# xiaoyeli/superlu_dist

Measured on AMD Instinct MI355X. Metric: LU factorization GFLOP/s (pdgstrf3d) + solve time, higher is better.
Workload: dtype f64

## Files before the change

__graft_entry__.py:

```python
import os, subprocess, sys

ROOT = os.path.dirname(os.path.abspath(__file__))
sys.path.insert(0, ROOT)
sys.path.insert(0, os.path.join(ROOT, "tests"))


def build():
    subprocess.check_call(["make", "-C", os.path.join(ROOT, "superlu_dist_amd", "csrc")])
    subprocess.check_call(["make", "-C", os.path.join(ROOT, "examples")])
    subprocess.check_call(["make", "-C", os.path.join(ROOT, "oracle")])
    ref_cfg = "/root/reference/SRC/include/superlu_dist_config.h"
    if os.path.isdir("/root/reference/SRC") and not os.path.exists(ref_cfg):
        print("build(): " + ref_cfg + " is absent (cmake-generated): the real reference is NOT built here; oracle/_ref* stay as they are", file=sys.stderr)
    if os.path.exists(ref_cfg):
        subprocess.check_call(["make", "-s", "-C", os.path.join(ROOT, "oracle", "ref")])
        subprocess.check_call(["make", "-s", "-C", os.path.join(ROOT, "oracle", "ref"), "ref64", "-j8"])
        if os.path.exists("/opt/conda/lib/libmkl_rt.so"):
            subprocess.check_call(["make", "-s", "-C", os.path.join(ROOT, "oracle", "ref"), "ref_mkl", "-j8"])
    import superlu_dist_amd
    from superlu_dist_amd import _lib
    _lib.load()


def smoke():
# ... 31 lines not shown
```

include/superlu_dist_amd.h:

```cpp
#ifndef SUPERLU_DIST_AMD_H
#define SUPERLU_DIST_AMD_H

#include <stdint.h>

#ifdef __cplusplus
extern "C" {
#endif

typedef int32_t sluamd_int_t;

#define SLUAMD_OK 0
#define SLUAMD_EINVAL (-1)
#define SLUAMD_ENODEVICE (-2)
#define SLUAMD_EHIP (-3)
#define SLUAMD_ENOMEM (-4)
#define SLUAMD_ESTRUCT (-5)

typedef struct sluamd_dLUview {
    int64_t n;
    int32_t nsupers;
    const sluamd_int_t *xsup;
    int32_t nprow, npcol, npdep;
    int32_t myrow, mycol, myzlayer;
    sluamd_int_t **Lrowind_bc_ptr;
// ... 83 lines not shown
int sluamd_pzgstrf3d(sluamd_handle_t h, double thresh, int *info);
int sluamd_zCopyLU2Host(sluamd_handle_t h, const sluamd_zLUview_t *lu);
int sluamd_pzgstrs3d(sluamd_handle_t h, sluamd_doublecomplex *x, int64_t ldx, int32_t nrhs);

#define SLUAMD_NOTRANS 0
#define SLUAMD_TRANS   1
#define SLUAMD_CONJ    2
int sluamd_pdgstrs3d_trans(sluamd_handle_t h, int trans, double *x, int64_t ldx, int32_t nrhs);
int sluamd_pdgstrs3d_trans_dev(sluamd_handle_t h, int trans, double *d_x, int64_t ldx, int32_t nrhs);
int sluamd_pzgstrs3d_trans(sluamd_handle_t h, int trans, sluamd_doublecomplex *x, int64_t ldx, int32_t nrhs);
int sluamd_pzgstrs3d_trans_dev(sluamd_handle_t h, int trans, sluamd_doublecomplex *d_x, int64_t ldx, int32_t nrhs);

void sluamd_dDestroyLUHandle(sluamd_handle_t h);

int sluamd_get_stats(sluamd_handle_t h, sluamd_stats_t *out);
int sluamd_setup_times(sluamd_handle_t h, char *buf, int32_t cap);
#define SLUAMD_PLAN_COLS 20
int sluamd_plan_table(sluamd_handle_t h, double *buf, int64_t cap_rows, int64_t *rows);
const char *sluamd_last_error(void);
int sluamd_device_count(void);
int64_t sluamd_device_pool_trim(int dev);
int sluamd_device_pci_bus_id(int dev, char *buf, int len);

typedef struct sluamd_symb_s *sluamd_symb_t;

int sluamd_dsymbfact(sluamd_symb_t *s, int64_t n, const sluamd_int_t *rowptr, const sluamd_int_t *colind,
                     const sluamd_int_t *perm_c, int32_t relax, int32_t maxsup, sluamd_int_t *perm_c_out);
int sluamd_dsymbfact_unsym(sluamd_symb_t *s, int64_t n, const sluamd_int_t *rowptr, const sluamd_int_t *colind,
                           const sluamd_int_t *perm_c, int32_t relax, int32_t maxsup, sluamd_int_t *perm_c_out);
int sluamd_order_nd(int64_t n, const sluamd_int_t *rowptr, const sluamd_int_t *colind, int32_t leaf, sluamd_int_t *perm_c);
// ... 106 lines not shown
```

superlu_dist_amd/_lib.py:

```python
import ctypes as C
import os

_HERE = os.path.dirname(os.path.abspath(__file__))
_SO = os.environ.get("SLUAMD_LIB") or os.path.join(_HERE, "libsluamd.so")

int_t = C.c_int32
P_int = C.POINTER(C.c_int32)
P_dbl = C.POINTER(C.c_double)


class LUView(C.Structure):
    _fields_ = [("n", C.c_int64), ("nsupers", C.c_int32), ("xsup", P_int),
                ("nprow", C.c_int32), ("npcol", C.c_int32), ("npdep", C.c_int32),
                ("myrow", C.c_int32), ("mycol", C.c_int32), ("myzlayer", C.c_int32),
                ("Lrowind_bc_ptr", C.POINTER(P_int)), ("Lnzval_bc_ptr", C.POINTER(P_dbl)),
                ("Ufstnz_br_ptr", C.POINTER(P_int)), ("Unzval_br_ptr", C.POINTER(P_dbl))]


class ForestView(C.Structure):
    _fields_ = [("maxLvl", C.c_int32), ("myTreeIdxs", P_int), ("myZeroTrIdxs", P_int),
                ("numForests", C.c_int32), ("nNodes", P_int), ("nodeList", C.POINTER(P_int))]


class Options(C.Structure):
# ... 69 lines not shown
    L.sluamd_dCreateLUHandleFromSymb.argtypes = [C.POINTER(C.c_void_p), C.c_void_p, P_int, P_int, P_dbl, P_int, C.POINTER(Options)]
    L.sluamd_dCreateLUHandleFromSymbGrid.argtypes = [C.POINTER(C.c_void_p), C.c_void_p, P_int, P_int, P_dbl, P_int, C.POINTER(Options),
                                                     P_int, C.c_void_p]
    L.sluamd_zCreateLUHandleFromSymbGrid.argtypes = [C.POINTER(C.c_void_p), C.c_void_p, P_int, P_int, C.c_void_p, P_int, C.POINTER(Options),
                                                     P_int, C.c_void_p]
    L.sluamd_dSetValues.argtypes = [C.c_void_p, C.POINTER(LUView)]
    L.sluamd_pdgstrf3d.argtypes = [C.c_void_p, C.c_double, P_int]
    L.sluamd_factor_info.argtypes = [C.c_void_p, P_int, P_int]
    L.sluamd_dCopyLU2Host.argtypes = [C.c_void_p, C.POINTER(LUView)]
    L.sluamd_pdgstrs3d.argtypes = [C.c_void_p, P_dbl, C.c_int64, C.c_int32]
    L.sluamd_pdgstrs3d_dev.argtypes = [C.c_void_p, C.c_void_p, C.c_int64, C.c_int32]
    L.sluamd_pdgstrs3d_dist.argtypes = [C.c_void_p, C.c_void_p, C.c_int64, C.c_int32, C.c_int64, C.c_int64, P_int, P_int]
    L.sluamd_pzgstrs3d_dist.argtypes = L.sluamd_pdgstrs3d_dist.argtypes
    L.sluamd_dDestroyLUHandle.argtypes = [C.c_void_p]
    L.sluamd_get_stats.argtypes = [C.c_void_p, C.POINTER(Stats)]
    L.sluamd_mfma_selftest.argtypes = [P_dbl, P_dbl, P_dbl]
    L.sluamd_dResetValues.argtypes = [C.c_void_p]
    L.sluamd_zCreateLUHandle.argtypes = L.sluamd_dCreateLUHandle.argtypes
    L.sluamd_zCreateLUHandleGrid.argtypes = L.sluamd_dCreateLUHandleGrid.argtypes
    L.sluamd_zSetValues.argtypes = [C.c_void_p, C.POINTER(LUView)]
    L.sluamd_zCopyLU2Host.argtypes = [C.c_void_p, C.POINTER(LUView)]
    L.sluamd_pzgstrf3d.argtypes = [C.c_void_p, C.c_double, P_int]
    L.sluamd_pzgstrs3d.argtypes = [C.c_void_p, C.c_void_p, C.c_int64, C.c_int32]
    L.sluamd_zCreateLUHandleFromSymb.argtypes = [C.POINTER(C.c_void_p), C.c_void_p, P_int, P_int, C.c_void_p, P_int, C.POINTER(Options)]
    L.sluamd_symb_partition.argtypes = [C.c_void_p, C.c_int32, P_int]
    L.sluamd_symb_grid_footprint.argtypes = [C.c_void_p, C.c_int32, C.c_int32, C.c_int32, P_int, C.POINTER(C.c_int64), C.POINTER(C.c_int64), C.POINTER(C.c_int64)]
    L.sluamd_set_profile.argtypes = [C.c_void_p, C.c_int]
    L.sluamd_setup_times.argtypes = [C.c_void_p, C.c_char_p, C.c_int32]
    L.sluamd_poisson3d.argtypes = [C.c_int32, C.c_int32, C.c_int32, P_int, P_int, P_dbl]
    L.sluamd_poisson3d.restype = C.c_int64
# ... 53 lines not shown
```

superlu_dist_amd/csrc/sluamd_api.cpp:

```cpp
#include <algorithm>
#include <cstdint>
#include <cstdlib>
#include <cstring>
#include "sluamd_comm.h"
#include "sluamd_plan.h"
#include "sluamd_refine.h"

using namespace sluamd;

namespace sluamd {

static int ensure_pinned(Handle *H)
{
    if (H->h_pinned) return 0;
    size_t want = (size_t) 64 << 20;
    if (const char *v = getenv("SLUAMD_PINNED_BYTES")) want = std::max<size_t>(256, (size_t) atoll(v) & ~(size_t) 15);
    HIPCHK(hipHostMalloc(&H->h_pinned, want, hipHostMallocDefault));
    H->pinned_bytes = want;
    return 0;
}

static int copy_values(Handle *H, const sluamd_dLUview_t *lu, int dir)
{
    const HostStruct &hs = H->hs;
// ... 620 lines not shown
                    double b = 0.0;
                    for (size_t a = zl + 1; a < H->forest_nodes.size(); ++a)
                        for (int k : H->forest_nodes[a]) {
                            if (H->grid.kcol(k) == H->grid.c) b += (double) (esz * H->hs.lval_len[k]);
                            if (H->grid.krow(k) == H->grid.r) b += (double) (esz * H->hs.uval_len[k]);
                        }
                    r[15] = send ? b : -b;
                }
            }
        }
    }
    *rows = n;
    return 0;
}

int sluamd_get_stats(sluamd_handle_t h, sluamd_stats_t *out)
{
    if (!h || !out) return SLUAMD_EINVAL;
    *out = h->H.st;
    return 0;
}

int sluamd_dCreateLUHandleFromSymb(sluamd_handle_t *out, sluamd_symb_t s, const sluamd_int_t *rowptr, const sluamd_int_t *colind,
                                   const double *nzval, const sluamd_int_t *perm_c_final, const sluamd_options_t *opt)
{
    return create_from_symb(out, s, rowptr, colind, nzval, perm_c_final, opt, Grid{}, nullptr, nullptr, false);
}

int sluamd_zCreateLUHandleFromSymb(sluamd_handle_t *out, sluamd_symb_t s, const sluamd_int_t *rowptr, const sluamd_int_t *colind,
                                   const sluamd_doublecomplex *nzval, const sluamd_int_t *perm_c_final, const sluamd_options_t *opt)
// ... 58 lines not shown
```

superlu_dist_amd/csrc/sluamd_factor.cpp:

```cpp
#include <algorithm>
#include <cstring>
#include "sluamd_comm.h"
#include "sluamd_plan.h"

namespace sluamd {

static void ev_begin(Handle *H, std::vector<std::pair<hipEvent_t, hipEvent_t>> &v, size_t &used, hipStream_t s)
{
    if (!H->profile) return;
    if (used == v.size()) { hipEvent_t a, b; hipEventCreate(&a); hipEventCreate(&b); v.emplace_back(a, b); }
    hipEventRecord(v[used].first, s);
}
static void ev_end(Handle *H, std::vector<std::pair<hipEvent_t, hipEvent_t>> &v, size_t &used, hipStream_t s)
{
    if (!H->profile) return;
    hipEventRecord(v[used].second, s);
    ++used;
}
static double ev_sum(std::vector<std::pair<hipEvent_t, hipEvent_t>> &v, size_t used)
{
    double tot = 0;
    for (size_t i = 0; i < used; ++i) { float ms = 0; hipEventElapsedTime(&ms, v[i].first, v[i].second); tot += ms; }
    return tot;
}
// ... 377 lines not shown
    return 0;
}

static hipEvent_t red_wait_event(const Handle *H, int64_t lend, int64_t uend)
{
    for (auto &e : H->red_events)
        if ((lend < 0 || e.lend >= lend) && (uend < 0 || e.uend >= uend)) return e.ev;
    return H->red_events.empty() ? nullptr : H->red_events.back().ev;
}

int run_factor(Handle *H, double thresh, int *info)
{
    HIPCHK(hipSetDevice(H->device));
    const Grid &g = H->grid;
    if (g.size() > 1 && !H->comm) { set_error("handle of a multi-rank grid has no communicator"); return SLUAMD_EINVAL; }
    int init[8] = {0x7fffffff, 0, 0, 0, 0, 0, 0, 0};
    HIPCHK(hipMemcpyAsync(H->d_info, init, sizeof(init), hipMemcpyHostToDevice, H->stream));
    H->st.num_launches = 0; H->st.schur_launches = 0; H->st.schur_tiles = 0;
    H->profile = H->opt.verbose >= 2 || H->env.profile;
    H->ev_schur_used = H->ev_panel_used = H->ev_xchg_used = H->ev_red_used = 0;
    H->schur_rec.clear();
    H->ev_pool_used = 0;
    H->red_pool_used = 0; H->red_events.clear();
    HIPCHK(hipEventRecord(H->ev0, H->stream));
    int rc = 0;
    for (size_t zl = 0; zl < H->sched.size(); ++zl) {
        if (H->z_active[zl]) {
            rc = run_factor_sched(H, H->sched[zl], thresh);
            if (rc) return rc;
        }
        if (g.Pz > 1) {
            ev_begin(H, H->ev_red, H->ev_red_used, H->stream);
            rc = reduce_ancestors(H, (int) zl);
            ev_end(H, H->ev_red, H->ev_red_used, H->stream);
            if (rc) return rc;
        }
    }
    if (H->red_all) { HIPCHK(hipStreamWaitEvent(H->stream, H->red_all, 0)); H->red_events.clear(); }
    HIPCHK(hipEventRecord(H->ev1, H->stream));
    int res[8];
    HIPCHK(hipMemcpyAsync(res, H->d_info, sizeof(res), hipMemcpyDeviceToHost, H->stream));
    HIPCHK(hipStreamSynchronize(H->stream));
    float ms = 0; HIPCHK(hipEventElapsedTime(&ms, H->ev0, H->ev1));
    H->st.t_factor_ms = ms;
    if (getenv("SLUAMD_EXP_COUNT")) fprintf(stderr, "[sluamd] K chunks of the Schur tiles (instrumented kernel build only): 128 x 128 clean %d other %d; 64 x 64 clean %d other %d\n", res[4], res[5], res[6], res[7]);
    H->dinv_ready = true; H->inv_ready = !H->env.trsm_panels && !H->z; H->factored = true;
    if (H->profile && H->env.profile_dump && H->schur_rec.size() == H->ev_schur_used)
        for (size_t i = 0; i < H->ev_schur_used; ++i) {
            float ems = 0; hipEventElapsedTime(&ems, H->ev_schur[i].first, H->ev_schur[i].second);
            const auto &r = H->schur_rec[i];
            fprintf(stderr, "SCHUR level %d pass %d big %d tiles %d max_nsupc %d ms %.4f\n", r.level, r.pass, r.big, r.ntiles, r.mx, ems);
        }
    H->st.t_schur_ms = H->profile ? ev_sum(H->ev_schur, H->ev_schur_used) : 0.0;
    H->st.t_schur_big_ms = 0.0;
    if (H->profile)
        for (size_t i = 0; i < H->ev_schur_used && i < H->ev_schur_big.size(); ++i)
            if (H->ev_schur_big[i]) { float ms = 0; hipEventElapsedTime(&ms, H->ev_schur[i].first, H->ev_schur[i].second); H->st.t_schur_big_ms += ms; }
    H->st.t_panel_ms = H->profile ? ev_sum(H->ev_panel, H->ev_panel_used) : 0.0;
    H->st.t_exchange_ms = H->profile ? ev_sum(H->ev_xchg, H->ev_xchg_used) : 0.0;
// ... 721 lines not shown
```

superlu_dist_amd/csrc/sluamd_internal.h:

```cpp
#pragma once
#include <cstdint>
#include <map>
#include <string>
#include <utility>
#include <vector>
#include <sluamd_rt.h>
#include "superlu_dist_amd.h"

namespace sluamd {

constexpr int BC_HEADER = 2;
constexpr int LB_DESCRIPTOR = 2;
constexpr int BR_HEADER = 3;
constexpr int UB_DESCRIPTOR = 2;
constexpr int DB = 32;
constexpr int KC = 16;

void set_error(const std::string &msg);
const std::string &get_error();

#define HIPCHK(expr)                                                                         \
    do {                                                                                     \
        hipError_t e_ = (expr);                                                              \
        if (e_ != hipSuccess) {                                                              \
// ... 230 lines not shown
    std::vector<std::vector<int>> forest_nodes;
    std::vector<uint8_t> z_active;
    std::vector<int> own_l_order, own_u_order;
    SplitMap split;
    hipStream_t stream = nullptr;
    hipStream_t pstream = nullptr;
    hipStream_t ustream = nullptr;
    hipStream_t u2stream = nullptr;
    hipStream_t rstream = nullptr;
    struct RedEv { int64_t lend, uend; hipEvent_t ev; };
    std::vector<RedEv> red_events;
    std::vector<hipEvent_t> red_pool; size_t red_pool_used = 0;
    hipEvent_t red_all = nullptr;
    std::vector<hipEvent_t> ev_pool;
    size_t ev_pool_used = 0;
    int *d_info = nullptr;
    double *d_x = nullptr; int64_t x_cap = 0;
    double *d_xtmp = nullptr; int64_t xtmp_cap = 0;
    double *d_w = nullptr; int64_t w_cap = 0;
    int64_t *d_apos = nullptr; double *d_aval = nullptr; int64_t a_nnz = 0;
    int *d_aent = nullptr; int64_t a_csr_nnz = -1;
    double *d_eq_r = nullptr, *d_eq_c = nullptr; bool eq_done = false, eq_row = false, eq_col = false;
    double *d_eq_work = nullptr; int64_t eq_work_cap = 0;
    int *d_rfs_rp = nullptr, *d_rfs_ci = nullptr, *d_rfs_pc = nullptr; double *d_rfs_av = nullptr;
    double *d_rfs_work = nullptr; unsigned long long *d_rfs_s = nullptr; int64_t rfs_nnz = 0;
    bool rfs_z = false;
    void *h_pinned = nullptr; size_t pinned_bytes = 0;
    bool z = false;
    bool dinv_ready = false;
    bool inv_ready = false;
// ... 106 lines not shown
```

superlu_dist_amd/csrc/sluamd_kernels.hip:

```cpp
#include <hip/hip_runtime.h>
#include <cassert>
#include <cstdio>
#include "sluamd_internal.h"

namespace sluamd {

typedef double d4 __attribute__((ext_vector_type(4)));

__device__ __forceinline__ int find_node(const int *__restrict__ prefix, int nn, int id)
{
    int lo = 0, hi = nn;
    while (hi - lo > 1) {
        int mid = (lo + hi) >> 1;
        if (prefix[mid] <= id) lo = mid; else hi = mid;
    }
    return lo;
}

#ifndef SLUAMD_FIND_WAVE
#define SLUAMD_FIND_WAVE 1
#endif
__device__ __forceinline__ int find_node_wave(const int *__restrict__ prefix, int nn, int id)
{
#if SLUAMD_FIND_WAVE
// ... 973 lines not shown
    if (threadIdx.x == 0) {
        q = fmax(fmax(red[0], red[1]), fmax(red[2], red[3]));
        atomicMax(s_out, (unsigned long long) __double_as_longlong(q));
    }
}

__global__ __launch_bounds__(256) void k_rfs_update(int n, const int *__restrict__ pc, const double *__restrict__ dx_perm,
                                                    double *__restrict__ x)
{
    const int i = blockIdx.x * 256 + threadIdx.x;
    if (i < n) x[i] += dx_perm[pc[i]];
}


typedef const volatile double __attribute__((address_space(3))) *lds_vdouble_t;
template <int RA, int CA, int LDL, int LDU, bool USW>
__device__ __forceinline__ void schur_chunk(const double *Lb, const double *Ub, int rm0, int cn0, int lane, d4 (&acc)[CA][RA], int pa)
{
#pragma unroll
    for (int k4 = 0; k4 < KC; k4 += 4) {
        const int kr = k4 + (lane >> 4);
        double a[CA], b[RA];
#pragma unroll
        for (int c = 0; c < CA; ++c) a[c] = USW ? ((lds_vdouble_t) Ub)[(pa ^ k4) + 256 * c] : Ub[kr * LDU + cn0 + 16 * c + (lane & 15)];
#pragma unroll
        for (int r = 0; r < RA; ++r) b[r] = USW ? ((lds_vdouble_t) Lb)[kr * LDL + rm0 + 16 * r + (lane & 15)] : Lb[kr * LDL + rm0 + 16 * r + (lane & 15)];
#pragma unroll
        for (int c = 0; c < CA; ++c)
#pragma unroll
            for (int r = 0; r < RA; ++r) acc[c][r] = __builtin_amdgcn_mfma_f64_16x16x4f64(a[c], b[r], acc[c][r], 0, 0, 0);
    }
}

#ifndef SLUAMD_EXP_EPI
#define SLUAMD_EXP_EPI 2
#endif
#ifndef SLUAMD_EXP_NOLOAD
#define SLUAMD_EXP_NOLOAD 0
#endif
#ifndef SLUAMD_EXP_VALU
#define SLUAMD_EXP_VALU 0
// ... 25 lines not shown
#ifdef SLUAMD_EXP_NODMAWAIT
__device__ __forceinline__ void lds_dma_wait() { asm volatile("" ::: "memory"); }
#else
__device__ __forceinline__ void lds_dma_wait() { asm volatile("s_waitcnt vmcnt(0)" ::: "memory"); }
#endif
__device__ __forceinline__ uint32_t lds_byte_addr(const void *p) { return (uint32_t) (uintptr_t) (__attribute__((address_space(3))) const void *) p; }
#ifndef SLUAMD_SCHUR_TOUCH
#define SLUAMD_SCHUR_TOUCH 0
#endif
#ifndef SLUAMD_SCHUR_TIGHT
#define SLUAMD_SCHUR_TIGHT 1
#endif
#ifndef SLUAMD_SCHUR_DMA
#define SLUAMD_SCHUR_DMA 1
#endif
#ifndef SLUAMD_SCHUR_CLEAN
#define SLUAMD_SCHUR_CLEAN 1
#endif
typedef double d2 __attribute__((ext_vector_type(2)));
typedef const d2 __attribute__((address_space(1), aligned(8))) *gd2_t;
typedef const char __attribute__((address_space(1))) *gbytes_t;
typedef const double __attribute__((address_space(1))) *gdouble_t;
__device__ __forceinline__ gbytes_t uniform_ptr(const double *p)
{
    const uint64_t v = (uint64_t) p;
    const uint32_t lo = __builtin_amdgcn_readfirstlane((uint32_t) v), hi = __builtin_amdgcn_readfirstlane((uint32_t) (v >> 32));
    return (gbytes_t) (((uint64_t) hi << 32) | lo);
}
#ifndef SCHUR64_WGS
#define SCHUR64_WGS 5
#endif
template <int TMv, int TNv, int NW, bool Z = false, int MM = 0, bool SK = false>
__global__ __launch_bounds__(NW * 64, (NW == 8 ? 4 : (TMv == 128 ? 2 : (Z ? 6 : SCHUR64_WGS)))) void k_schur(DevTables T, const int *__restrict__ nodes,
                                                                    const int *__restrict__ prefix, int nn, int id_base,
                                                                    int ntiles, int *__restrict__ info,
                                                                    const int4 *__restrict__ ulist, int prio,
                                                                    const int *__restrict__ tmaps, const int *__restrict__ xoff)
{
    constexpr int LDL = TMv + 16;
    constexpr int LDU = TNv + 17;
    constexpr int NT = NW * 64;
    constexpr int WR = (NW == 8) ? 4 : 2, WC = 2;
    constexpr int NBR = TMv / (16 * WR), NBC = TNv / (16 * WC);
    constexpr int LQ = TMv * KC / NT, UQ = TNv * KC / NT;
    constexpr int LKS = NT / TMv;
    constexpr int UJS = NT / 16;
    constexpr int ZS = Z ? 2 : 1;
    static_assert(!Z || (LKS % 2 == 0 && KC % 2 == 0), "complex L loader: the parity of a thread's k must be constant");
    constexpr int NBUF = (TMv == 64 && SCHUR64_WGS > 4) ? 1 : 2;
    __shared__ double Ls[NBUF][KC * LDL];
    constexpr bool USW = SLUAMD_SCHUR_FETCH3 && !Z;
    __shared__ __attribute__((aligned(16))) double Us[NBUF][USW ? KC * TNv : KC * LDU];
    auto uidx = [](int k, int c) { return USW ? c * 16 + ((((k >> 1) ^ ((c >> 1) & 7)) << 1) | (k & 1)) : k * LDU + c; };
    __shared__ int s_ind[256 + 8];
    __shared__ int s_rowmap[TMv];
    __shared__ int s_colmap[TNv];
    __shared__ int s_cptr[TNv];
    __shared__ int s_lead[TNv];
    __shared__ int s_cptr2[TNv];
    __shared__ int s_lead2[TNv];
    __shared__ int s_jj[TNv];
    __shared__ int s_dinfo[1];
    __shared__ int s_sink[(SLUAMD_SCHUR_TOUCH == 2 && TMv == 128) ? NW * 64 : 1];
    constexpr int HDR = 64;
// ... 192 lines not shown
                rec[HDR + TMv + TNv + t] = s_cptr[t];
                rec[HDR + TMv + 2 * TNv + t] = s_lead[t];
            }
            return;
        }
    }
    int nprev = 0;
    if (MM == 2) nprev = Z ? 0 : s_hdr[16];
    else if (!Z && T.fuse_prev) { while (nprev < 3 && T.fuse_prev[3 * k + nprev] >= 0) ++nprev; }
    double touch0 = 0.0, touch1 = 0.0;

    const int wave = __builtin_amdgcn_readfirstlane(tid >> 6), lane = tid & 63;
    const int rm0 = ((wave + bid) % WR) * (TMv / WR), cn0 = (wave / WR) * (TNv / WC);
    const bool wave_on = rm0 < nr && cn0 < nc;
    const int pa = uidx(lane >> 4, cn0 + (lane & 15));
    d4 acc[NBC][NBR];
#pragma unroll
    for (int a = 0; a < NBC; ++a)
#pragma unroll
        for (int b = 0; b < NBR; ++b) acc[a][b] = (d4){0.0, 0.0, 0.0, 0.0};

    const int li = tid % TMv, lk = tid / TMv;
    const int uk = tid & 15, uj = tid >> 4;
    double pl[LQ], pu[UQ];
    const int *cpS = s_cptr, *ldS = s_lead;
    bool lrow_ok = li < nr;
    const int zoff = Z ? ((li ^ lk) & 1) : 0;
    const double zsgn = (Z && !(li & 1) && (lk & 1)) ? -1.0 : 1.0;
    const int lrow0 = Z ? (li & ~1) + zoff : li;
    int ns_s = ZS * ns, lda_s = lda;
    const double *Lrow = Lp + lrow0, *Uvs = Uv;
    const double *Lsrc = Lp;
    uint32_t lvo = (uint32_t) (lrow0 + lk * lda) << 3;
    constexpr bool F3 = SLUAMD_SCHUR_FETCH3 && !Z;
    constexpr int LRP = TMv / 2, LKS3 = NT / LRP, LQ3 = KC / LKS3, UJS3 = NT / 8, UQ3 = TNv / UJS3;
    const int li2 = tid % LRP, lk3 = tid / LRP, uk2 = tid & 7, uj3 = tid >> 3;
    d2 wl[F3 ? LQ3 : 1], wu[F3 ? UQ3 : 1];
    bool un0[F3 ? UQ3 : 1], un1[F3 ? UQ3 : 1];
    bool l_has0 = 2 * li2 < nr, l_has1 = 2 * li2 + 1 < nr;
    bool lon[F3 ? LQ3 : 1];
    uint32_t lvo3 = (uint32_t) (2 * li2 + lk3 * lda) << 3;
    bool rows_ok3 = true;
    auto l3_source = [&](int ra0, int ra1, int ldas) {
        l_has0 = ra0 >= 0; l_has1 = ra1 >= 0;
        lvo3 = (uint32_t) ((l_has0 ? ra0 : max(ra1, 0)) + lk3 * ldas) << 3;
        const bool p0 = 2 * li2 < nr, p1 = 2 * li2 + 1 < nr;
        rows_ok3 = !p0 || (l_has0 && (!p1 || ra1 == ra0 + 1));
    };
    auto fetch3 = [&](int k0) {
        const gbytes_t Lb0 = uniform_ptr(Lsrc), Ub0 = uniform_ptr(Uvs);
#pragma unroll
// ... 9 lines not shown
        const int kg = k0 + 2 * uk2;
#pragma unroll
        for (int q = 0; q < UQ3; ++q) {
            un0[q] = kg >= ldq[q] && kg < ns_s;
            un1[q] = kg + 1 >= ldq[q] && kg + 1 < ns_s;
            const uint32_t uvo = (un0[q] || un1[q]) ? (uint32_t) (cpq[q] + max(kg - ldq[q], 0)) << 3 : 0;
            wu[q] = *(gd2_t) (Ub0 + (uint64_t) uvo);
        }
    };
    auto stash3 = [&](int buf) {
#pragma unroll
        for (int q = 0; q < LQ3; ++q) {
            d2 v;
            v.x = (lon[q] && l_has0) ? wl[q].x : 0.0;
            v.y = (lon[q] && l_has1) ? (l_has0 ? wl[q].y : wl[q].x) : 0.0;
            *(d2 *) &Ls[buf][(lk3 + LKS3 * q) * LDL + 2 * li2] = v;
        }
#pragma unroll
        for (int q = 0; q < UQ3; ++q) {
            d2 y;
            y.x = un0[q] ? wu[q].x : 0.0; y.y = un1[q] ? (un0[q] ? wu[q].y : wu[q].x) : 0.0;
            *(d2 *) &Us[buf][uidx(2 * uk2, uj3 + UJS3 * q)] = y;
        }
    };

    bool clean = false;
    uint32_t uvoc[F3 ? UQ3 : 1];
    int kbeg0 = 0;
    bool cur_fast = false;
    i32x4 rsL = {0, 0, 0, 0}, rsU = {0, 0, 0, 0};
    auto source_clean = [&](int kb, bool rows_ok) {
        int ok = rows_ok ? 1 : 0;
#pragma unroll
        for (int q = 0; q < UQ3; ++q) {
            const int c = uj3 + UJS3 * q;
            const int ld = ldS[c], cp = cpS[c];
            if (c < nc && (ld > kb || cp > 0x0F000000)) ok = 0;
            uvoc[q] = (c < nc) ? (uint32_t) (cp - ld + kb + 2 * (uk2 ^ ((c >> 1) & 7))) << 3 : (uint32_t) (2 * uk2) << 3;
        }
        kbeg0 = kb;
        if ((uint64_t) (uint32_t) ns_s * (uint64_t) (uint32_t) lda_s > 0x0F000000ull) ok = 0;
        clean = __syncthreads_and(ok) != 0;
        if (clean) { rsL = buffer_rsrc(Lsrc); rsU = buffer_rsrc(Uvs); }
    };
    constexpr bool DMA = F3 && TMv == 128 && NBUF == 2 && SLUAMD_SCHUR_DMA && SLUAMD_SCHUR_CLEAN;
    static_assert(!DMA || (LRP == 64 && UJS3 * UQ3 == TNv), "LDS-DMA loader: one panel column / eight tile columns per wave and load");
    auto fetch_clean = [&](int k0, int tb) {
#ifdef SLUAMD_EXP_NOWAIT
#pragma unroll
        for (int q = 0; q < LQ3; ++q) asm volatile("" :: "v"(wl[q]));
#pragma unroll
        for (int q = 0; q < UQ3; ++q) asm volatile("" :: "v"(wu[q]));
#endif
        if (DMA) {
#pragma unroll
            for (int q = 0; q < LQ3; ++q)
                lds_dma_16(rsL, __builtin_amdgcn_readfirstlane(lds_byte_addr(&Ls[tb][(wave + LKS3 * q) * LDL])), (int) lvo3, (int) ((uint32_t) (k0 + LKS3 * q) * (uint32_t) lda_s << 3));
#pragma unroll
            for (int q = 0; q < UQ3; ++q)
                lds_dma_16(rsU, __builtin_amdgcn_readfirstlane(lds_byte_addr(&Us[tb][(8 * wave + UJS3 * q) * 16])), (int) uvoc[q], (int) ((uint32_t) (k0 - kbeg0) << 3));
            return;
        }
#pragma unroll
        for (int q = 0; q < LQ3; ++q)
            wl[q] = __builtin_bit_cast(d2, llvm_amdgcn_raw_buffer_load_i32x4(rsL, (int) lvo3, (int) ((uint32_t) (k0 + LKS3 * q) * (uint32_t) lda_s << 3), 0));
#pragma unroll
        for (int q = 0; q < UQ3; ++q) wu[q] = __builtin_bit_cast(d2, llvm_amdgcn_raw_buffer_load_i32x4(rsU, (int) uvoc[q], (int) ((uint32_t) (k0 - kbeg0) << 3), 0));
    };
    auto stash_clean = [&](int buf) {
        if (DMA) { lds_dma_wait(); return; }
#ifdef SLUAMD_EXP_NOSTASH
        return;
#endif
#ifdef SLUAMD_EXP_NOWAIT
        const d2 cst = {1.0 + 1e-9 * tid, 1.0 - 1e-9 * tid};
#pragma unroll
        for (int q = 0; q < LQ3; ++q) *(d2 *) &Ls[buf][(lk3 + LKS3 * q) * LDL + 2 * li2] = cst;
#pragma unroll
        for (int q = 0; q < UQ3; ++q) {
            *(d2 *) &Us[buf][(uj3 + UJS3 * q) * 16 + 2 * uk2] = cst;
        }
        return;
#endif
#pragma unroll
        for (int q = 0; q < LQ3; ++q) *(d2 *) &Ls[buf][(lk3 + LKS3 * q) * LDL + 2 * li2] = wl[q];
#pragma unroll
        for (int q = 0; q < UQ3; ++q) {
            *(d2 *) &Us[buf][(uj3 + UJS3 * q) * 16 + 2 * uk2] = wu[q];
        }
    };

    auto fetch_into = [&](double *pl, double *pu, int k0, bool restart = false) {
#if SLUAMD_EXP_NOLOAD
        if (SLUAMD_EXP_NOLOAD == 1 || (SLUAMD_EXP_NOLOAD <= 3 && (SLUAMD_EXP_NOLOAD == 2) == restart)) {
#pragma unroll
            for (int q = 0; q < LQ; ++q) pl[q] = 1.0 + 1e-9 * (k0 + q);
#pragma unroll
            for (int q = 0; q < UQ; ++q) pu[q] = 1.0 - 1e-9 * (k0 + q);
            return;
        }
// ... 122 lines not shown
            kend = min(ns_s, kbeg + c1 * KC); kbeg += c0 * KC;
            if (kbeg >= kend) continue;
        }
        kend_cur = kend;
        const int ktouch = (src == nprev && has_dst) ? max(kbeg, kbeg + ((kend - 1 - kbeg) / KC - 1) * KC) : -1;
#if SLUAMD_SCHUR_TIGHT
        if (DMA && clean && !SLUAMD_EXP_NOLOAD && SLUAMD_SCHUR_TOUCH == 0) {
            const int nfull = (kend - kbeg) / KC;
            if (nfull > 0) {
                fetch_clean(kbeg, buf);
                lds_dma_wait();
                __syncthreads();
                for (int c = 0; c < nfull; ++c) {
                    const bool more = c + 1 < nfull;
                    if (more) fetch_clean(kbeg + KC, buf ^ 1);
                    if (wave_on) schur_chunk<NBR, NBC, LDL, LDU, USW>(Ls[buf], Us[buf], rm0, cn0, lane, acc, pa);
                    if (more) lds_dma_wait();
                    buf ^= 1;
                    kbeg += KC;
                    __syncthreads();
                }
#ifdef SLUAMD_EXP_COUNT
                cnt_fast += nfull;
#endif
                if (kbeg >= kend) continue;
            }
        }
#endif
        fetch(kbeg, buf, true);
        stash(buf);
        __syncthreads();
// ... 13 lines not shown
                if (DMA) {
                    const double *t0 = (id0 < TNv * RG && c0 < nc && g0 * 16 < nr) ? dst + s_colmap[c0] + s_rowmap[g0 * 16] : dst;
                    const double *t1 = (id1 < TNv * RG && c1 < nc && g1 * 16 < nr) ? dst + s_colmap[c1] + s_rowmap[g1 * 16] : dst;
                    const uint32_t sink = __builtin_amdgcn_readfirstlane(lds_byte_addr(&s_sink[wave * 64]));
                    unsigned keep;
                    asm volatile("s_mov_b32 %0, m0\n\ts_mov_b32 m0, %3\n\ts_nop 0\n\tglobal_load_lds_dword %1, off\n\tglobal_load_lds_dword %2, off\n\ts_mov_b32 m0, %0"
                                 : "=&s"(keep) : "v"(t0), "v"(t1), "s"(sink) : "memory");
                } else
#endif
                {
                if (id0 < TNv * RG && c0 < nc && g0 * 16 < nr) touch0 = dst[s_colmap[c0] + s_rowmap[g0 * 16]];
                if (id1 < TNv * RG && c1 < nc && g1 * 16 < nr) touch1 = dst[s_colmap[c1] + s_rowmap[g1 * 16]];
                }
            }
            const double *Lb = Ls[buf], *Ub = Us[buf];
            if (wave_on) schur_chunk<NBR, NBC, LDL, LDU, USW>(Lb, Ub, rm0, cn0, lane, acc, pa);
            if (NBUF == 2) { if (more) stash(buf ^ 1); buf ^= 1; }
            else if (more) { __syncthreads(); stash(0); }
            __syncthreads();
        }
    }

    if (DMA && SLUAMD_SCHUR_TOUCH == 2) lds_dma_wait();
#ifdef SLUAMD_EXP_COUNT
    if (tid == 0 && TMv == 128) { atomicAdd(&info[4], cnt_fast); atomicAdd(&info[5], cnt_slow); }
    if (tid == 0 && TMv == 64) { atomicAdd(&info[6], cnt_fast); atomicAdd(&info[7], cnt_slow); }
#endif
#if SLUAMD_EXP_VALU
    if (__builtin_expect((dummy0 ^ dummy1 ^ dummy2 ^ dummy3) == 0x7fffffff && tid == 777, 0)) atomicAdd(&info[3], 1);
#endif
    if (!has_dst) return;
    if (__builtin_expect(touch0 == 1.2345e-300 && touch1 == 1.2345e-300, 0)) atomicAdd(&info[3], 1);
#if SLUAMD_EXP_EPI == 0
    {
        double keep = 0.0;
#pragma unroll
        for (int ci = 0; ci < NBC; ++ci)
#pragma unroll
            for (int ri = 0; ri < NBR; ++ri) keep += (acc[ci][ri][0] + acc[ci][ri][1]) + (acc[ci][ri][2] + acc[ci][ri][3]);
        if (__builtin_expect(keep == 1.2345e-300, 0)) atomicAdd(&info[3], 1);
        return;
// ... 1420 lines not shown
```

superlu_dist_amd/csrc/sluamd_plan.cpp:

```cpp
#include <algorithm>
#include <atomic>
#include <cstdio>
#include <cstring>
#include <numeric>
#include <queue>
#include <functional>
#include <cmath>
#include "sluamd_comm.h"
#include "sluamd_plan.h"

namespace sluamd {

static inline int nsupc_of(const HostStruct &hs, int k) { return hs.xsup[k + 1] - hs.xsup[k]; }

static void dag_levels(const SlotInput &in, const std::vector<int> &list, int ns, std::vector<int> &lvl, int &nlevels)
{
    lvl.assign(ns, -1);
    for (int k : list) lvl[k] = 0;
    int maxl = 0;
    for (int k : list) {
        const int l1 = lvl[k] + 1;
        for (int g : in.succ[k]) if (lvl[g] >= 0 && lvl[g] < l1) lvl[g] = l1;
        maxl = std::max(maxl, lvl[k]);
    }
// ... 1584 lines not shown
    if (!H->h_lrow_near.empty()) {
        uint8_t *p0, *p1;
        if (upload(K, H->h_lrow_near, &p0) || upload(K, H->h_ucol_near, &p1)) return SLUAMD_EHIP;
        T.lrow_near = p0; T.ucol_near = p1;
        std::vector<uint8_t>().swap(H->h_lrow_near); std::vector<uint8_t>().swap(H->h_ucol_near);
    }
    if (H->fused_pairs) {
        int *p0, *p1, *p2, *p3, *p4, *p5;
        if (upload(K, H->h_fuse_prev, &p0) || upload(K, H->h_defer, &p1) || upload(K, H->h_pair_roff, &p2) ||
            upload(K, H->h_pair_coff, &p3) || upload(K, H->h_pair_rowmap, &p4) || upload(K, H->h_pair_colinfo, &p5)) return SLUAMD_EHIP;
        T.fuse_prev = p0; T.defer = p1; T.pair_roff = p2; T.pair_coff = p3; T.pair_rowmap = p4; T.pair_colinfo = p5;
    }
    H->st.reserved_i = H->fused_pairs;
    H->st.schur_tiles = 0;
    for (auto &S : H->sched) H->st.schur_tiles += (int64_t) S.ulist.size();
    HIPCHK(hipMalloc((void **) &H->d_info, 8 * sizeof(int)));
    if (H->z) { std::vector<int> zero(std::max(ns, 1), 0); if (upload(K, zero, &H->d_ztickets)) return SLUAMD_EHIP; }
    rc = eng::setup();
    if (rc) return rc;
    H->setup.lap("upload.rest");
    arena_job.th.join();
    if (arena_rc == 1) {
        (void) hipGetLastError();
        size_t fr = 0, tot = 0;
        hipMemGetInfo(&fr, &tot);
        char msg[512];
        snprintf(msg, sizeof msg, "hipMalloc of the value arena failed: rank (%d,%d,%d) of the %d x %d x %d grid needs %.1f GB (own L/U slots %.1f GB + exchange scratch %.1f GB) "
                 "and %.1f GB of %.1f GB are free on device %d -- use a larger process grid (scripts/capacity.py prints the per-rank storage of a grid)",
                 H->grid.r, H->grid.c, H->grid.z, H->grid.Pr, H->grid.Pc, H->grid.Pz, esz * (double) H->arena_len / 1e9, esz * (double) H->own_len / 1e9,
                 esz * (double) (H->arena_len - H->own_len) / 1e9, fr / 1e9, tot / 1e9, H->device);
        set_error(msg);
// ... 17 lines not shown
```

superlu_dist_amd/driver.py:

```python
import ctypes as C
import numpy as np
from . import _lib
from ._lib import LUView, ForestView, Options, Stats, P_int, P_dbl


def _pi(a):
    return a.ctypes.data_as(P_int)


def _pd(a):
    return a.ctypes.data_as(P_dbl)


class FlatStore:

    def __init__(self, n, xsup, Lrowind_off, Lrowind, Lnzval_off, Lnzval, Ufstnz_off, Ufstnz, Unzval_off, Unzval,
                 grid=(1, 1, 1), coords=(0, 0, 0)):
        self.n = int(n)
        self.xsup = np.ascontiguousarray(xsup, dtype=np.int32)
        self.nsupers = len(self.xsup) - 1
        self.Lrowind_off = np.asarray(Lrowind_off, dtype=np.int64)
        self.Lrowind = np.ascontiguousarray(Lrowind, dtype=np.int32)
        self.Lnzval_off = np.asarray(Lnzval_off, dtype=np.int64)
        self.z = bool(np.iscomplexobj(Lnzval) or np.iscomplexobj(Unzval))
# ... 257 lines not shown
    def scalings(self):
        return _scalings(self._h, self.n)

    def gssvx_solve(self, b, trans="N", refine=False):
        return _gssvx_solve(self._h, self.z, b, trans, refine)

    def gssvx_solve_dev(self, d_b, ldb, d_x, ldx, nrhs, trans="N", refine=False):
        return _gssvx_solve_dev(self._h, self.z, d_b, ldb, d_x, ldx, nrhs, trans, refine)

    def set_profile(self, on=True):
        _lib.load().sluamd_set_profile(self._h, int(on))

    def stats(self):
        s = Stats()
        _lib.load().sluamd_get_stats(self._h, C.byref(s))
        return {f[0]: getattr(s, f[0]) for f in Stats._fields_}

    def plan_table(self):
        return plan_table(self._h)

    def diag_inv(self, k, ns):
        li = np.zeros((ns, ns), order="F"); ui = np.zeros((ns, ns), order="F")
        _lib.check(_lib.load().sluamd_dGetDiagInv(self._h, int(k), _pd(li), _pd(ui)), "sluamd_dGetDiagInv")
        return li, ui

    def setup_times(self):
        buf = C.create_string_buffer(4096)
        if _lib.load().sluamd_setup_times(self._h, buf, 4096):
            return {}
        out = {}
        for tok in buf.value.decode().split(";"):
# ... 168 lines not shown
```

Before: 48180.

## Extend LDS-DMA loading to 64-row Schur tiles with swizzled unpadded L stage

Lets the 64-row, 4-wave Schur update kernel load L and U panels with the asynchronous LDS-DMA path used by the 128-row tiles. The L stage is unpadded and XOR-swizzled to avoid bank conflicts, and the kernel is double-buffered. The occupancy hint for this variant drops to 4 workgroups to make room for the second buffer. It also adds counters for clean and mixed K-chunks, exposed through a new stats API. The aim is to overlap global-to-LDS traffic with MFMA work on the many small Schur tiles, at the cost of occupancy and extra LDS.

```diff
diff --git a/__graft_entry__.py b/__graft_entry__.py
--- a/__graft_entry__.py
+++ b/__graft_entry__.py
@@ -6,7 +6,7 @@
 
 
 def build():
-    subprocess.check_call(["make", "-C", os.path.join(ROOT, "superlu_dist_amd", "csrc")])
+    subprocess.check_call(["make", "-j2", "-C", os.path.join(ROOT, "superlu_dist_amd", "csrc")])
     subprocess.check_call(["make", "-C", os.path.join(ROOT, "examples")])
     subprocess.check_call(["make", "-C", os.path.join(ROOT, "oracle")])
     ref_cfg = "/root/reference/SRC/include/superlu_dist_config.h"
diff --git a/include/superlu_dist_amd.h b/include/superlu_dist_amd.h
--- a/include/superlu_dist_amd.h
+++ b/include/superlu_dist_amd.h
@@ -121,6 +121,7 @@
 void sluamd_dDestroyLUHandle(sluamd_handle_t h);
 
 int sluamd_get_stats(sluamd_handle_t h, sluamd_stats_t *out);
+int sluamd_schur_chunk_counts(sluamd_handle_t h, int64_t out[5]);
 int sluamd_setup_times(sluamd_handle_t h, char *buf, int32_t cap);
 #define SLUAMD_PLAN_COLS 20
 int sluamd_plan_table(sluamd_handle_t h, double *buf, int64_t cap_rows, int64_t *rows);
diff --git a/superlu_dist_amd/_lib.py b/superlu_dist_amd/_lib.py
--- a/superlu_dist_amd/_lib.py
+++ b/superlu_dist_amd/_lib.py
@@ -107,6 +107,8 @@
     L.sluamd_pzgstrs3d_dist.argtypes = L.sluamd_pdgstrs3d_dist.argtypes
     L.sluamd_dDestroyLUHandle.argtypes = [C.c_void_p]
     L.sluamd_get_stats.argtypes = [C.c_void_p, C.POINTER(Stats)]
+    if hasattr(L, "sluamd_schur_chunk_counts"):
+        L.sluamd_schur_chunk_counts.argtypes = [C.c_void_p, C.POINTER(C.c_int64)]
     L.sluamd_mfma_selftest.argtypes = [P_dbl, P_dbl, P_dbl]
     L.sluamd_dResetValues.argtypes = [C.c_void_p]
     L.sluamd_zCreateLUHandle.argtypes = L.sluamd_dCreateLUHandle.argtypes
diff --git a/superlu_dist_amd/csrc/sluamd_api.cpp b/superlu_dist_amd/csrc/sluamd_api.cpp
--- a/superlu_dist_amd/csrc/sluamd_api.cpp
+++ b/superlu_dist_amd/csrc/sluamd_api.cpp
@@ -658,6 +658,13 @@
     return 0;
 }
 
+int sluamd_schur_chunk_counts(sluamd_handle_t h, int64_t out[5])
+{
+    if (!h || !out) return SLUAMD_EINVAL;
+    for (int i = 0; i < 5; ++i) out[i] = h->H.schur_chunks[i];
+    return 0;
+}
+
 int sluamd_get_stats(sluamd_handle_t h, sluamd_stats_t *out)
 {
     if (!h || !out) return SLUAMD_EINVAL;
diff --git a/superlu_dist_amd/csrc/sluamd_factor.cpp b/superlu_dist_amd/csrc/sluamd_factor.cpp
--- a/superlu_dist_amd/csrc/sluamd_factor.cpp
+++ b/superlu_dist_amd/csrc/sluamd_factor.cpp
@@ -415,7 +415,7 @@
     HIPCHK(hipSetDevice(H->device));
     const Grid &g = H->grid;
     if (g.size() > 1 && !H->comm) { set_error("handle of a multi-rank grid has no communicator"); return SLUAMD_EINVAL; }
-    int init[8] = {0x7fffffff, 0, 0, 0, 0, 0, 0, 0};
+    int init[12] = {0x7fffffff, 0, 0, 0, 0, 0, 0, 0, 0, 0, 0, 0};
     HIPCHK(hipMemcpyAsync(H->d_info, init, sizeof(init), hipMemcpyHostToDevice, H->stream));
     H->st.num_launches = 0; H->st.schur_launches = 0; H->st.schur_tiles = 0;
     H->profile = H->opt.verbose >= 2 || H->env.profile;
@@ -439,11 +439,12 @@
     }
     if (H->red_all) { HIPCHK(hipStreamWaitEvent(H->stream, H->red_all, 0)); H->red_events.clear(); }
     HIPCHK(hipEventRecord(H->ev1, H->stream));
-    int res[8];
+    int res[12];
     HIPCHK(hipMemcpyAsync(res, H->d_info, sizeof(res), hipMemcpyDeviceToHost, H->stream));
     HIPCHK(hipStreamSynchronize(H->stream));
     float ms = 0; HIPCHK(hipEventElapsedTime(&ms, H->ev0, H->ev1));
     H->st.t_factor_ms = ms;
+    for (int i = 0; i < 5; ++i) H->schur_chunks[i] = H->z ? 0 : res[4 + i];
     if (getenv("SLUAMD_EXP_COUNT")) fprintf(stderr, "[sluamd] K chunks of the Schur tiles (instrumented kernel build only): 128 x 128 clean %d other %d; 64 x 64 clean %d other %d\n", res[4], res[5], res[6], res[7]);
     H->dinv_ready = true; H->inv_ready = !H->env.trsm_panels && !H->z; H->factored = true;
     if (H->profile && H->env.profile_dump && H->schur_rec.size() == H->ev_schur_used)
diff --git a/superlu_dist_amd/csrc/sluamd_internal.h b/superlu_dist_amd/csrc/sluamd_internal.h
--- a/superlu_dist_amd/csrc/sluamd_internal.h
+++ b/superlu_dist_amd/csrc/sluamd_internal.h
@@ -268,6 +268,7 @@
     hipEvent_t red_all = nullptr;
     std::vector<hipEvent_t> ev_pool;
     size_t ev_pool_used = 0;
+    int schur_chunks[5] = {0, 0, 0, 0, 0};
     int *d_info = nullptr;
     double *d_x = nullptr; int64_t x_cap = 0;
     double *d_xtmp = nullptr; int64_t xtmp_cap = 0;
diff --git a/superlu_dist_amd/csrc/sluamd_kernels.hip b/superlu_dist_amd/csrc/sluamd_kernels.hip
--- a/superlu_dist_amd/csrc/sluamd_kernels.hip
+++ b/superlu_dist_amd/csrc/sluamd_kernels.hip
@@ -1011,9 +1011,10 @@
 
 
 typedef const volatile double __attribute__((address_space(3))) *lds_vdouble_t;
-template <int RA, int CA, int LDL, int LDU, bool USW>
-__device__ __forceinline__ void schur_chunk(const double *Lb, const double *Ub, int rm0, int cn0, int lane, d4 (&acc)[CA][RA], int pa)
-{
+template <int RA, int CA, int LDL, int LDU, bool USW, bool LSW = false>
+__device__ __forceinline__ void schur_chunk(const double *Lb, const double *Ub, int rm0, int cn0, int lane, d4 (&acc)[CA][RA], int pa, int pb0 = 0, int pb1 = 0)
+{
+    static_assert(!LSW || (USW && RA == 2), "swizzled L stage: two row blocks per wave");
 #pragma unroll
     for (int k4 = 0; k4 < KC; k4 += 4) {
         const int kr = k4 + (lane >> 4);
@@ -1021,7 +1022,7 @@
 #pragma unroll
         for (int c = 0; c < CA; ++c) a[c] = USW ? ((lds_vdouble_t) Ub)[(pa ^ k4) + 256 * c] : Ub[kr * LDU + cn0 + 16 * c + (lane & 15)];
 #pragma unroll
-        for (int r = 0; r < RA; ++r) b[r] = USW ? ((lds_vdouble_t) Lb)[kr * LDL + rm0 + 16 * r + (lane & 15)] : Lb[kr * LDL + rm0 + 16 * r + (lane & 15)];
+        for (int r = 0; r < RA; ++r) b[r] = LSW ? ((lds_vdouble_t) Lb)[(r ? pb1 : pb0) + k4 * LDL] : (USW ? ((lds_vdouble_t) Lb)[kr * LDL + rm0 + 16 * r + (lane & 15)] : Lb[kr * LDL + rm0 + 16 * r + (lane & 15)]);
 #pragma unroll
         for (int c = 0; c < CA; ++c)
 #pragma unroll
@@ -1077,6 +1078,9 @@
 #ifndef SLUAMD_SCHUR_DMA
 #define SLUAMD_SCHUR_DMA 1
 #endif
+#ifndef SLUAMD_SCHUR64_DMA
+#define SLUAMD_SCHUR64_DMA 1
+#endif
 #ifndef SLUAMD_SCHUR_CLEAN
 #define SLUAMD_SCHUR_CLEAN 1
 #endif
@@ -1093,14 +1097,17 @@
 #ifndef SCHUR64_WGS
 #define SCHUR64_WGS 5
 #endif
+template <int TMv, int NW, bool Z>
+constexpr bool schur64_dma() { return SLUAMD_SCHUR64_DMA && SLUAMD_SCHUR_DMA && SLUAMD_SCHUR_CLEAN && SLUAMD_SCHUR_FETCH3 && !SLUAMD_EXP_NOLOAD && !Z && TMv == 64 && NW == 4; }
 template <int TMv, int TNv, int NW, bool Z = false, int MM = 0, bool SK = false>
-__global__ __launch_bounds__(NW * 64, (NW == 8 ? 4 : (TMv == 128 ? 2 : (Z ? 6 : SCHUR64_WGS)))) void k_schur(DevTables T, const int *__restrict__ nodes,
+__global__ __launch_bounds__(NW * 64, (NW == 8 ? 4 : (TMv == 128 ? 2 : (Z ? 6 : (schur64_dma<TMv, NW, Z>() ? 4 : SCHUR64_WGS))))) void k_schur(DevTables T, const int *__restrict__ nodes,
                                                                     const int *__restrict__ prefix, int nn, int id_base,
                                                                     int ntiles, int *__restrict__ info,
                                                                     const int4 *__restrict__ ulist, int prio,
                                                                     const int *__restrict__ tmaps, const int *__restrict__ xoff)
 {
-    constexpr int LDL = TMv + 16;
+    constexpr bool D64 = schur64_dma<TMv, NW, Z>();
+    constexpr int LDL = D64 ? TMv : TMv + 16;
     constexpr int LDU = TNv + 17;
     constexpr int NT = NW * 64;
     constexpr int WR = (NW == 8) ? 4 : 2, WC = 2;
@@ -1110,7 +1117,7 @@
     constexpr int UJS = NT / 16;
     constexpr int ZS = Z ? 2 : 1;
     static_assert(!Z || (LKS % 2 == 0 && KC % 2 == 0), "complex L loader: the parity of a thread's k must be constant");
-    constexpr int NBUF = (TMv == 64 && SCHUR64_WGS > 4) ? 1 : 2;
+    constexpr int NBUF = (TMv == 64 && !D64 && SCHUR64_WGS > 4) ? 1 : 2;
     __shared__ double Ls[NBUF][KC * LDL];
     constexpr bool USW = SLUAMD_SCHUR_FETCH3 && !Z;
     __shared__ __attribute__((aligned(16))) double Us[NBUF][USW ? KC * TNv : KC * LDU];
@@ -1333,6 +1340,7 @@
     const int rm0 = ((wave + bid) % WR) * (TMv / WR), cn0 = (wave / WR) * (TNv / WC);
     const bool wave_on = rm0 < nr && cn0 < nc;
     const int pa = uidx(lane >> 4, cn0 + (lane & 15));
+    const int pb0 = (lane >> 4) * LDL + rm0 + (lane & 15) + ((lane & 16) ? 16 : 0), pb1 = (lane >> 4) * LDL + rm0 + (lane & 15) + ((lane & 16) ? 0 : 16);
     d4 acc[NBC][NBR];
 #pragma unroll
     for (int a = 0; a < NBC; ++a)
@@ -1353,7 +1361,9 @@
     uint32_t lvo = (uint32_t) (lrow0 + lk * lda) << 3;
     constexpr bool F3 = SLUAMD_SCHUR_FETCH3 && !Z;
     constexpr int LRP = TMv / 2, LKS3 = NT / LRP, LQ3 = KC / LKS3, UJS3 = NT / 8, UQ3 = TNv / UJS3;
-    const int li2 = tid % LRP, lk3 = tid / LRP, uk2 = tid & 7, uj3 = tid >> 3;
+    const int ls2 = tid % LRP, lk3 = tid / LRP, uk2 = tid & 7, uj3 = tid >> 3;
+    const int li2 = D64 ? ls2 ^ ((lk3 & 1) << 3) : ls2;
+    static_assert(!D64 || (LKS3 % 2 == 0 && LRP == 32), "64-row LDS-DMA loader: a thread's panel columns keep their parity");
     d2 wl[F3 ? LQ3 : 1], wu[F3 ? UQ3 : 1];
     bool un0[F3 ? UQ3 : 1], un1[F3 ? UQ3 : 1];
     bool l_has0 = 2 * li2 < nr, l_has1 = 2 * li2 + 1 < nr;
@@ -1393,7 +1403,7 @@
             d2 v;
             v.x = (lon[q] && l_has0) ? wl[q].x : 0.0;
             v.y = (lon[q] && l_has1) ? (l_has0 ? wl[q].y : wl[q].x) : 0.0;
-            *(d2 *) &Ls[buf][(lk3 + LKS3 * q) * LDL + 2 * li2] = v;
+            *(d2 *) &Ls[buf][(lk3 + LKS3 * q) * LDL + 2 * ls2] = v;
         }
 #pragma unroll
         for (int q = 0; q < UQ3; ++q) {
@@ -1422,8 +1432,10 @@
         clean = __syncthreads_and(ok) != 0;
         if (clean) { rsL = buffer_rsrc(Lsrc); rsU = buffer_rsrc(Uvs); }
     };
-    constexpr bool DMA = F3 && TMv == 128 && NBUF == 2 && SLUAMD_SCHUR_DMA && SLUAMD_SCHUR_CLEAN;
-    static_assert(!DMA || (LRP == 64 && UJS3 * UQ3 == TNv), "LDS-DMA loader: one panel column / eight tile columns per wave and load");
+    constexpr bool DMA = F3 && (TMv == 128 || D64) && NBUF == 2 && SLUAMD_SCHUR_DMA && SLUAMD_SCHUR_CLEAN;
+    constexpr int LCW = 64 / LRP;
+    static_assert(!DMA || (((LRP == 64 && LCW == 1) || (LRP == 32 && LCW == 2 && LDL == 2 * LRP)) && LCW * NW == LKS3 && UJS3 * UQ3 == TNv && UJS3 == 8 * NW),
+                  "LDS-DMA loader: one panel column (128-row tiles) or two adjacent unpadded ones (64-row tiles) and eight tile columns per wave and load");
     auto fetch_clean = [&](int k0, int tb) {
 #ifdef SLUAMD_EXP_NOWAIT
 #pragma unroll
@@ -1434,7 +1446,7 @@
         if (DMA) {
 #pragma unroll
             for (int q = 0; q < LQ3; ++q)
-                lds_dma_16(rsL, __builtin_amdgcn_readfirstlane(lds_byte_addr(&Ls[tb][(wave + LKS3 * q) * LDL])), (int) lvo3, (int) ((uint32_t) (k0 + LKS3 * q) * (uint32_t) lda_s << 3));
+                lds_dma_16(rsL, __builtin_amdgcn_readfirstlane(lds_byte_addr(&Ls[tb][(LCW * wave + LKS3 * q) * LDL])), (int) lvo3, (int) ((uint32_t) (k0 + LKS3 * q) * (uint32_t) lda_s << 3));
 #pragma unroll
             for (int q = 0; q < UQ3; ++q)
                 lds_dma_16(rsU, __builtin_amdgcn_readfirstlane(lds_byte_addr(&Us[tb][(8 * wave + UJS3 * q) * 16])), (int) uvoc[q], (int) ((uint32_t) (k0 - kbeg0) << 3));
@@ -1454,7 +1466,7 @@
 #ifdef SLUAMD_EXP_NOWAIT
         const d2 cst = {1.0 + 1e-9 * tid, 1.0 - 1e-9 * tid};
 #pragma unroll
-        for (int q = 0; q < LQ3; ++q) *(d2 *) &Ls[buf][(lk3 + LKS3 * q) * LDL + 2 * li2] = cst;
+        for (int q = 0; q < LQ3; ++q) *(d2 *) &Ls[buf][(lk3 + LKS3 * q) * LDL + 2 * ls2] = cst;
 #pragma unroll
         for (int q = 0; q < UQ3; ++q) {
             *(d2 *) &Us[buf][(uj3 + UJS3 * q) * 16 + 2 * uk2] = cst;
@@ -1462,7 +1474,7 @@
         return;
 #endif
 #pragma unroll
-        for (int q = 0; q < LQ3; ++q) *(d2 *) &Ls[buf][(lk3 + LKS3 * q) * LDL + 2 * li2] = wl[q];
+        for (int q = 0; q < LQ3; ++q) *(d2 *) &Ls[buf][(lk3 + LKS3 * q) * LDL + 2 * ls2] = wl[q];
 #pragma unroll
         for (int q = 0; q < UQ3; ++q) {
             *(d2 *) &Us[buf][(uj3 + UJS3 * q) * 16 + 2 * uk2] = wu[q];
@@ -1615,7 +1627,7 @@
                 for (int c = 0; c < nfull; ++c) {
                     const bool more = c + 1 < nfull;
                     if (more) fetch_clean(kbeg + KC, buf ^ 1);
-                    if (wave_on) schur_chunk<NBR, NBC, LDL, LDU, USW>(Ls[buf], Us[buf], rm0, cn0, lane, acc, pa);
+                    if (wave_on) schur_chunk<NBR, NBC, LDL, LDU, USW, D64>(Ls[buf], Us[buf], rm0, cn0, lane, acc, pa, pb0, pb1);
                     if (more) lds_dma_wait();
                     buf ^= 1;
                     kbeg += KC;
@@ -1659,7 +1671,7 @@
                 }
             }
             const double *Lb = Ls[buf], *Ub = Us[buf];
-            if (wave_on) schur_chunk<NBR, NBC, LDL, LDU, USW>(Lb, Ub, rm0, cn0, lane, acc, pa);
+            if (wave_on) schur_chunk<NBR, NBC, LDL, LDU, USW, D64>(Lb, Ub, rm0, cn0, lane, acc, pa, pb0, pb1);
             if (NBUF == 2) { if (more) stash(buf ^ 1); buf ^= 1; }
             else if (more) { __syncthreads(); stash(0); }
             __syncthreads();
@@ -1669,7 +1681,7 @@
     if (DMA && SLUAMD_SCHUR_TOUCH == 2) lds_dma_wait();
 #ifdef SLUAMD_EXP_COUNT
     if (tid == 0 && TMv == 128) { atomicAdd(&info[4], cnt_fast); atomicAdd(&info[5], cnt_slow); }
-    if (tid == 0 && TMv == 64) { atomicAdd(&info[6], cnt_fast); atomicAdd(&info[7], cnt_slow); }
+    if (tid == 0 && TMv == 64) { atomicAdd(&info[6], cnt_fast); atomicAdd(&info[7], cnt_slow); if (cnt_fast) atomicAdd(&info[8], cnt_slow); }
 #endif
 #if SLUAMD_EXP_VALU
     if (__builtin_expect((dummy0 ^ dummy1 ^ dummy2 ^ dummy3) == 0x7fffffff && tid == 777, 0)) atomicAdd(&info[3], 1);
diff --git a/superlu_dist_amd/csrc/sluamd_plan.cpp b/superlu_dist_amd/csrc/sluamd_plan.cpp
--- a/superlu_dist_amd/csrc/sluamd_plan.cpp
+++ b/superlu_dist_amd/csrc/sluamd_plan.cpp
@@ -1622,7 +1622,7 @@
     H->st.reserved_i = H->fused_pairs;
     H->st.schur_tiles = 0;
     for (auto &S : H->sched) H->st.schur_tiles += (int64_t) S.ulist.size();
-    HIPCHK(hipMalloc((void **) &H->d_info, 8 * sizeof(int)));
+    HIPCHK(hipMalloc((void **) &H->d_info, 12 * sizeof(int)));
     if (H->z) { std::vector<int> zero(std::max(ns, 1), 0); if (upload(K, zero, &H->d_ztickets)) return SLUAMD_EHIP; }
     rc = eng::setup();
     if (rc) return rc;
diff --git a/superlu_dist_amd/driver.py b/superlu_dist_amd/driver.py
--- a/superlu_dist_amd/driver.py
+++ b/superlu_dist_amd/driver.py
@@ -295,7 +295,14 @@
     def stats(self):
         s = Stats()
         _lib.load().sluamd_get_stats(self._h, C.byref(s))
-        return {f[0]: getattr(s, f[0]) for f in Stats._fields_}
+        st = {f[0]: getattr(s, f[0]) for f in Stats._fields_}
+        L = _lib.load()
+        if hasattr(L, "sluamd_schur_chunk_counts"):
+            cnt = (C.c_int64 * 5)()
+            L.sluamd_schur_chunk_counts(self._h, cnt)
+            st.update(zip(("schur_chunks_big_clean", "schur_chunks_big_other", "schur_chunks_small_clean", "schur_chunks_small_other", "schur_chunks_small_mixed"),
+                          (int(v) for v in cnt)))
+        return st
 
     def plan_table(self):
         return plan_table(self._h)
```

Result: no change. 48550 (median of 6 runs) (+0.8%).
